# Soldann/MORB_SLAM

Hardware: AMD Instinct MI355X
Metric: stereo frames/sec ORB extract+match (752x480, 1200 feat = BASELINE configs[1]) (higher is better)
Workload: dtype u8; 1 GPU; BASELINE configs[1]: EuRoC-shaped stereo 752x480, 1200 feat: ORBextractor x2 + ComputeStereoMatches + ComputeBoW (synthetic k=10 L=6 vocabulary) + SearchByBoW vs previous frame; steps_in_flight=2, extract_streams=1, parallelism=frames dealt round-robin over 1 GPU(s)

## Files before the change

### morb_slam_amd/csrc/matcher.hip

```cpp
#include <hip/hip_runtime.h>

#include <algorithm>
#include <cstdlib>
#include <cstring>
#include <memory>
#include <vector>

#include "common.h"
#include "internal_abi.h"
#include "wave.h"
#include "extractor_internal.h"

using namespace morb;

namespace {

constexpr int TH_HIGH = 100, TH_LOW = 50, HISTO_LENGTH = 30;
constexpr int EDGE_ = 19;

struct Desc { uint32_t w[8]; };

__device__ __forceinline__ Desc load_desc(const uint8_t* p) {
  Desc d;
  const uint4* q = reinterpret_cast<const uint4*>(p);
// ... 325 lines not shown
      const int r = t / 3, c4 = (t - r * 3) * 4;
      pRow[j] = r - 5; pCol[j] = c4 - 5; pLds[j] = r * 12 + c4;
    } else {
      const int t2 = min(t, 98) - 33, r = t2 / 6, c4 = (t2 - r * 6) * 4;
      pRow[j] = r - 5; pCol[j] = c4 - 10; pLds[j] = 11 * 12 + r * 24 + c4;
    }
  }
  const uint64_t doMask = __ballot(cDo);
  const uint32_t cOffLlo = (uint32_t)cOffL, cOffLhi = (uint32_t)(cOffL >> 32), cOffRlo = (uint32_t)cOffR, cOffRhi = (uint32_t)(cOffR >> 32);
  uint8_t* patch = reinterpret_cast<uint8_t*>(pairs);
  int rS = -1, rInc = 0;
  float rD1 = 0.f, rD3 = 0.f;
  const int dy = min(lane & 15, 10);
  for (int q0 = 0; q0 < KQ; q0 += 4) {
    if (((doMask >> q0) & 15ull) == 0) continue;
    uint32_t pv[4][2];
#pragma unroll
    for (int k = 0; k < 4; ++k) {
      const int q = q0 + k;
      pv[k][0] = pv[k][1] = 0;
      if ((doMask >> q) & 1ull) {
        const unsigned long long oL = ((unsigned long long)(uint32_t)__builtin_amdgcn_readlane((int)cOffLhi, q) << 32) | (uint32_t)__builtin_amdgcn_readlane((int)cOffLlo, q);
        const unsigned long long oR = ((unsigned long long)(uint32_t)__builtin_amdgcn_readlane((int)cOffRhi, q) << 32) | (uint32_t)__builtin_amdgcn_readlane((int)cOffRlo, q);
        const int ps = __builtin_amdgcn_readlane(cPs, q);
#pragma unroll
        for (int j = 0; j < 2; ++j)
          if (pAct[j]) pv[k][j] = load_u32_unaligned(pyr + (pLeft[j] ? oL : oR) + (ptrdiff_t)pRow[j] * ps + pCol[j]);
      }
    }
    WAVE_SYNC();
#pragma unroll
    for (int k = 0; k < 4; ++k) {
      if (!((doMask >> (q0 + k)) & 1ull)) continue;
#pragma unroll
      for (int j = 0; j < 2; ++j)
        if (pAct[j]) *reinterpret_cast<uint32_t*>(patch + k * SM_PATCH + pLds[j]) = pv[k][j];
    }
    WAVE_SYNC();
#pragma unroll
    for (int k = 0; k < 4; ++k) {
      const int q = q0 + k;
      if (!((doMask >> q) & 1ull)) continue;
      const uint8_t* Lp = patch + k * SM_PATCH;
      const uint8_t* Rp = Lp + 11 * 12;
      const uint32_t l0 = *reinterpret_cast<const uint32_t*>(Lp + dy * 12), l1 = *reinterpret_cast<const uint32_t*>(Lp + dy * 12 + 4),
                     l2 = *reinterpret_cast<const uint32_t*>(Lp + dy * 12 + 8) & 0x00FFFFFFu;
      uint32_t bestKey = 0xFFFFFFFFu;
      int sums[12];
#pragma unroll
      for (int r = 0; r < 3; ++r) {
        const int sh = min(r * 4 + (lane >> 4), 10);
        const uint8_t* rp = Rp + dy * 24 + (sh & ~3);
        const uint32_t w0 = *reinterpret_cast<const uint32_t*>(rp), w1 = *reinterpret_cast<const uint32_t*>(rp + 4),
                       w2 = *reinterpret_cast<const uint32_t*>(rp + 8), w3 = *reinterpret_cast<const uint32_t*>(rp + 12);
        const uint32_t bsh = (uint32_t)(sh & 3);
        const uint32_t r0 = __builtin_amdgcn_alignbyte(w1, w0, bsh), r1 = __builtin_amdgcn_alignbyte(w2, w1, bsh),
                       r2 = __builtin_amdgcn_alignbyte(w3, w2, bsh) & 0x00FFFFFFu;
        int sv = (int)__builtin_amdgcn_sad_u8(l2, r2, __builtin_amdgcn_sad_u8(l1, r1, __builtin_amdgcn_sad_u8(l0, r0, 0u)));
        if ((lane & 15) > 10) sv = 0;
        sv += __builtin_amdgcn_update_dpp(0, sv, 0x111, 0xf, 0xf, true);
        sv += __builtin_amdgcn_update_dpp(0, sv, 0x112, 0xf, 0xf, true);
        sv += __builtin_amdgcn_update_dpp(0, sv, 0x114, 0xf, 0xf, true);
        sv += __builtin_amdgcn_update_dpp(0, sv, 0x118, 0xf, 0xf, true);
#pragma unroll
        for (int j = 0; j < 4; ++j) {
          sums[r * 4 + j] = __builtin_amdgcn_readlane(sv, 16 * j + 15);
          if (r * 4 + j < 11) {
            const uint32_t key = ((uint32_t)sums[r * 4 + j] << 4) | (uint32_t)(r * 4 + j);
            bestKey = key < bestKey ? key : bestKey;
          }
        }
      }
      const int bestS = (int)(bestKey >> 4), bi = (int)(bestKey & 15u);
      int s1 = 0, s3 = 0;
#pragma unroll
      for (int i = 0; i < 11; ++i) { s1 = (i == bi - 1) ? sums[i] : s1; s3 = (i == bi + 1) ? sums[i] : s3; }
      if (lane == q) { rS = bestS; rInc = bi - 5; rD1 = (float)s1; rD3 = (float)s3; }
    }
  }
  if (lane < KQ) {
    const int iL = iL0 + lane * 4 + wv;
    if (iL < cap) {
      float outU = -1.0f, outD = -1.0f;
      int outS = -1;
      if (cDo) {
        const int bestinc = rInc, bestS = rS;
        if (!(bestinc == -5 || bestinc == 5)) {
          const float dist1 = rD1, dist2 = (float)bestS, dist3 = rD3;
          const float deltaR = (dist1 - dist3) / (2.0f * (dist1 + dist3 - 2.0f * dist2));
          if (!(deltaR < -1 || deltaR > 1)) {
            float bestuR = sg.scale[cLvl & 15] * ((float)cUR0 + (float)bestinc + deltaR);
            float disparity = cUL - bestuR;
            if (disparity >= 0.f && disparity < maxD) {
              if (disparity <= 0) {
                disparity = 0.01f;
                bestuR = (float)((double)cUL - 0.01);
              }
              outD = mbf / disparity;
              outU = bestuR;
              outS = bestS;
            }
          }
        }
      }
      const size_t o = (size_t)f * cap + iL;
      uRight[o] = outU; depth[o] = outD; sadDist[o] = outS;
    }
  }
}

constexpr int SMED_V = 8;
template <int SMED_WAVES>
__global__ __launch_bounds__(64 * SMED_WAVES) void k_stereo_median(const int* __restrict__ count, int cap, float* __restrict__ uRight,
                                                       float* __restrict__ depth, const int* __restrict__ sadDist) {
  constexpr int NT = 64 * SMED_WAVES;
  const int f = blockIdx.x, tid = threadIdx.x;
  const int NL = count[2 * f];
  const size_t o = (size_t)f * cap;
  const bool inRegs = NL <= NT * SMED_V;
  int dv[SMED_V];
#pragma unroll
  for (int j = 0; j < SMED_V; ++j) { const int i = tid + j * NT; dv[j] = (inRegs && i < NL) ? sadDist[o + i] : -1; }
  int n = 0;
  if (inRegs) {
#pragma unroll
    for (int j = 0; j < SMED_V; ++j) n += dv[j] >= 0 ? 1 : 0;
  } else {
    for (int i = tid; i < NL; i += NT) n += sadDist[o + i] >= 0 ? 1 : 0;
  }
  __shared__ int red[2][SMED_WAVES];
  int phase = 0;
  auto blockSum = [&](int v) -> int {
    v = wave_sum(v);
    if ((tid & 63) == 0) red[phase][tid >> 6] = v;
    __syncthreads();
    int t = 0;
#pragma unroll
    for (int q = 0; q < SMED_WAVES; ++q) t += red[phase][q];
    phase ^= 1;
    return t;
  };
  const int total = blockSum(n);
  if (total == 0) return;
  const int k = total / 2;
  int lo = 0, hi = 121 * 255;
  while (lo < hi) {
    const int mid = (lo + hi) >> 1;
    int c = 0;
    if (inRegs) {
#pragma unroll
      for (int j = 0; j < SMED_V; ++j) c += (dv[j] >= 0 && dv[j] <= mid) ? 1 : 0;
    } else {
      for (int i = tid; i < NL; i += NT) { const int d = sadDist[o + i]; c += (d >= 0 && d <= mid) ? 1 : 0; }
    }
    c = blockSum(c);
    if (c > k) hi = mid; else lo = mid + 1;
  }
  const float median = (float)lo;
  const float thDist = 1.5f * 1.4f * median;
  if (inRegs) {
#pragma unroll
    for (int j = 0; j < SMED_V; ++j) {
      const int i = tid + j * NT;
      if (dv[j] >= 0 && !((float)dv[j] < thDist)) { uRight[o + i] = -1; depth[o + i] = -1; }
    }
  } else {
    for (int i = tid; i < NL; i += NT) {
      const int d = sadDist[o + i];
      if (d >= 0 && !((float)d < thDist)) { uRight[o + i] = -1; depth[o + i] = -1; }
    }
  }
}

__device__ __forceinline__ int quad_sum(int v) {
  v += __builtin_amdgcn_update_dpp(0, v, 0xB1, 0xF, 0xF, false);
  v += __builtin_amdgcn_update_dpp(0, v, 0x4E, 0xF, 0xF, false);
  return v;
}
__global__ __launch_bounds__(256) void k_bow_transform(const uint8_t* __restrict__ feat, const int* __restrict__ count,
                                                       int cap, const uint8_t* __restrict__ nodeDesc,
                                                       const int* __restrict__ firstChild, int k, int L, int levelsup,
                                                       int* __restrict__ wordId, int* __restrict__ nodeId,
                                                       const int* __restrict__ childCount) {
  const int img = blockIdx.y, t = blockIdx.x * 256 + threadIdx.x, i = t >> 2, sub = t & 3;
  if (i >= cap) return;
  const size_t o = (size_t)img * cap + i;
  if (i >= count[img]) { if (sub == 0) { wordId[o] = -1; nodeId[o] = -1; } return; }
  const uint2 d = *reinterpret_cast<const uint2*>(feat + o * 32 + sub * 8);
  const uint8_t* nd = nodeDesc + sub * 8;
  const int nid_level = L - levelsup;
  int final_id = 0, level = 0, nid = 0;
  do {
    ++level;
    const int c0 = firstChild[final_id];
    const int nc = childCount ? childCount[final_id] : k;
    int best = c0, bestd = 0x7fffffff;
    constexpr int CH = 5;
    for (int cb = c0; cb < c0 + nc; cb += CH) {
      uint2 tc[CH];
#pragma unroll
      for (int j = 0; j < CH; ++j) tc[j] = *reinterpret_cast<const uint2*>(nd + (size_t)min(cb + j, c0 + nc - 1) * 32);
#pragma unroll
      for (int j = 0; j < CH; ++j) {
        const int dd = quad_sum(__popc(d.x ^ tc[j].x) + __popc(d.y ^ tc[j].y));
        if (dd < bestd) { bestd = dd; best = min(cb + j, c0 + nc - 1); }
      }
    }
    final_id = best;
    if (level == nid_level) nid = final_id;
  } while (firstChild[final_id] >= 0);
  if (sub == 0) { wordId[o] = final_id; nodeId[o] = nid; }
}

constexpr int BT_K = 10, BT_N1 = BT_K, BT_N2 = BT_K * BT_K, BT_N3 = BT_K * BT_K * BT_K, BT_SLOTS = BT_N1 + BT_N2 + BT_N3;
template <int NLV> struct BtLds {
  static constexpr int SLOTS = NLV == 3 ? BT_SLOTS : BT_N1 + BT_N2;
  uint2 desc[SLOTS][4];
  int id[SLOTS];
  int fc[SLOTS];
  uint16_t nc[SLOTS];
};
template <int NLV>
__global__ __launch_bounds__(256) void k_bow_transform_lds(const uint8_t* __restrict__ feat, const int* __restrict__ count, int cap, int nimg,
                                                           const uint8_t* __restrict__ nodeDesc, const int* __restrict__ firstChild, int k,
                                                           int L, int levelsup, int* __restrict__ wordId, int* __restrict__ nodeId,
                                                           const int* __restrict__ childCount) {
  extern __shared__ __align__(16) uint8_t btRaw[];
  BtLds<NLV>& S = *reinterpret_cast<BtLds<NLV>*>(btRaw);
  const int tid = threadIdx.x;
  const int fc0 = firstChild[0], nc0 = childCount ? childCount[0] : k;
  auto stage = [&](int slot, int parentFc, int parentNc, int j) {
    int id = -1, fc = -1, nc = 0;
    if (parentFc >= 0 && j < parentNc) {
      id = parentFc + j;
      fc = firstChild[id];
      nc = fc >= 0 ? (childCount ? childCount[id] : k) : 0;
      const uint4* src = reinterpret_cast<const uint4*>(nodeDesc + (size_t)id * 32);
      const uint4 a = src[0], b = src[1];
      S.desc[slot][0] = make_uint2(a.x, a.y); S.desc[slot][1] = make_uint2(a.z, a.w);
      S.desc[slot][2] = make_uint2(b.x, b.y); S.desc[slot][3] = make_uint2(b.z, b.w);
    }
    S.id[slot] = id; S.fc[slot] = fc; S.nc[slot] = (uint16_t)min(nc, 0xFFFF);
  };
  if (tid < BT_N1) stage(tid, nc0 <= BT_K ? fc0 : -1, nc0, tid);
  __syncthreads();
  if (tid < BT_N2) { const int a = tid / BT_K; stage(BT_N1 + tid, S.nc[a] <= BT_K ? S.fc[a] : -1, S.nc[a], tid % BT_K); }
  __syncthreads();
  if (NLV == 3) for (int t = tid; t < BT_N3; t += 256) { const int ab = t / BT_K; stage(BT_N1 + BT_N2 + t, S.nc[BT_N1 + ab] <= BT_K ? S.fc[BT_N1 + ab] : -1, S.nc[BT_N1 + ab], t % BT_K); }
  __syncthreads();
  const int sub = tid & 3, nid_level = L - levelsup;
  const int chunksPerImg = (cap + 63) / 64, nChunks = chunksPerImg * nimg;
  const uint8_t* nd = nodeDesc + sub * 8;
  for (int ch = blockIdx.x; ch < nChunks; ch += gridDim.x) {
    const int img = ch / chunksPerImg, i = (ch - img * chunksPerImg) * 64 + (tid >> 2);
    if (i >= cap) continue;
    const size_t o = (size_t)img * cap + i;
    if (i >= count[img]) { if (sub == 0) { wordId[o] = -1; nodeId[o] = -1; } continue; }
    const uint2 d = *reinterpret_cast<const uint2*>(feat + o * 32 + sub * 8);
    int final_id = 0, level = 0, nid = 0;
    int slotBase = 0, nc = nc0, path = 0;
    bool leaf = fc0 < 0;
#pragma unroll
    for (int lv = 0; lv < NLV; ++lv) {
      if (leaf || nc > BT_K) break;
      ++level;
      int best = 0, bestd = 0x7fffffff;
      for (int j = 0; j < nc; ++j) {
        const uint2 tc = S.desc[slotBase + j][sub];
        const int dd = quad_sum(__popc(d.x ^ tc.x) + __popc(d.y ^ tc.y));
        if (dd < bestd) { bestd = dd; best = j; }
      }
      const int slot = slotBase + best;
      final_id = S.id[slot];
      if (level == nid_level) nid = final_id;
      leaf = S.fc[slot] < 0;
      nc = S.nc[slot];
      path = path * BT_K + best;
      slotBase = (lv == 0 ? BT_N1 : BT_N1 + BT_N2) + path * BT_K;
    }
    while (!leaf) {
      ++level;
      const int c0 = firstChild[final_id];
      const int ncg = childCount ? childCount[final_id] : k;
      int best = c0, bestd = 0x7fffffff;
      constexpr int CH = 5;
      for (int cb = c0; cb < c0 + ncg; cb += CH) {
        uint2 tc[CH];
#pragma unroll
        for (int j = 0; j < CH; ++j) tc[j] = *reinterpret_cast<const uint2*>(nd + (size_t)min(cb + j, c0 + ncg - 1) * 32);
#pragma unroll
        for (int j = 0; j < CH; ++j) {
          const int dd = quad_sum(__popc(d.x ^ tc[j].x) + __popc(d.y ^ tc[j].y));
          if (dd < bestd) { bestd = dd; best = min(cb + j, c0 + ncg - 1); }
        }
      }
      final_id = best;
      if (level == nid_level) nid = final_id;
      leaf = firstChild[final_id] < 0;
    }
    if (sub == 0) { wordId[o] = final_id; nodeId[o] = nid; }
  }
}

__global__ __launch_bounds__(1024) void k_bow_sort(const int* __restrict__ node, const int* __restrict__ count, int cap,
                                                   int P, unsigned long long* __restrict__ sorted) {
  extern __shared__ unsigned long long skeys[];
  const int img = blockIdx.x, tid = threadIdx.x, NT = blockDim.x;
  const int n = count[img];
  if (n == 0) {
    for (int i = tid; i < cap; i += NT) sorted[(size_t)img * cap + i] = ~0ull;
    return;
  }
  for (int i = tid; i < P; i += NT) {
    unsigned long long k = ~0ull;
    if (i < n) {
      const int nd = node[(size_t)img * cap + i];
      if (nd >= 0) k = ((unsigned long long)(unsigned)nd << 32) | (unsigned)i;
    }
    skeys[i] = k;
  }
  __syncthreads();
  const bool onePass = P / 2 <= NT;
  for (int k = 2; k <= P; k <<= 1)
    for (int j = k >> 1; j > 0; j >>= 1) {
      for (int l = tid; l < P / 2; l += NT) {
        const int i = ((l & ~(j - 1)) << 1) | (l & (j - 1)), ixj = i | j;
        const unsigned long long a = skeys[i], b = skeys[ixj];
        const bool up = (i & k) == 0;
        if ((a > b) == up) { skeys[i] = b; skeys[ixj] = a; }
      }
      const int jn = j > 1 ? j >> 1 : k;
      if (onePass && jn < 64 && j < 64) { __builtin_amdgcn_fence(__ATOMIC_SEQ_CST, "wavefront"); __builtin_amdgcn_wave_barrier(); }
      else __syncthreads();
    }
  for (int i = tid; i < cap; i += NT) sorted[(size_t)img * cap + i] = i < P ? skeys[i] : ~0ull;
}

#ifdef MORB_FAST_TIMING
__device__ unsigned long long g_bowTrace[16384 * 4];
#define BOW_MARK(k) do { if (lane == 0 && bw_ < 16384) g_bowTrace[bw_ * 4 + (k)] = wall_clock64(); } while (0)
#else
#define BOW_MARK(k)
#endif
constexpr int BM_NB = 25;
constexpr int BM_FJ = 4;
__device__ __forceinline__ unsigned wave_min_u32(unsigned v) { return morbwave::min_u32(v); }
__global__ __launch_bounds__(256) void k_bow_match(const unsigned long long* __restrict__ sortedKF,
                                                   const unsigned long long* __restrict__ sortedF,
                                                   const int* __restrict__ nKFv, const int* __restrict__ nFv, int cap,
                                                   const uint8_t* __restrict__ descKF, const uint8_t* __restrict__ hasMP,
                                                   const morb_keypoint* __restrict__ kpsKF,
                                                   const uint8_t* __restrict__ descF, const morb_keypoint* __restrict__ kpsF,
                                                   const int* __restrict__ kfImg, const int* __restrict__ fImg,
                                                   float nnratio, int* __restrict__ matchF, int* __restrict__ binF,
                                                   const int* __restrict__ nLeftv,
                                                   const uint8_t* __restrict__ hasMP2, const int* __restrict__ nValidv,
                                                   int* __restrict__ matched2) {
  extern __shared__ __align__(16) unsigned long long bowLds[];
#ifdef MORB_FAST_TIMING
  const int bw_ = (blockIdx.y * gridDim.x + blockIdx.x) * 4 + (threadIdx.x >> 6);
  if ((threadIdx.x & 63) == 0 && bw_ < 16384) g_bowTrace[bw_ * 4] = wall_clock64();
#endif
  unsigned long long* sk = bowLds;
  unsigned long long* sf = bowLds + cap;
  const int pair = blockIdx.y, tid = threadIdx.x, lane = tid & 63, wv = tid >> 6;
  const int ik = kfImg[pair], jf = fImg[pair];
  const int nKF = nKFv[ik], nF = nFv[jf];
  const bool fish = nLeftv != nullptr && nLeftv[pair] >= 0;
  const int nLeft = fish ? nLeftv[pair] : 0x7fffffff;
  const bool kfkf = hasMP2 != nullptr;
  const int nValid1 = (kfkf && nValidv) ? nValidv[ik] : 0x7fffffff, nValid2 = (kfkf && nValidv) ? nValidv[jf] : 0x7fffffff;
  const int thLow = kfkf ? TH_LOW - 1 : TH_LOW;
  {
    const unsigned long long* gk = sortedKF + (size_t)ik * cap;
    const unsigned long long* gf = sortedF + (size_t)jf * cap;
    for (int i0 = 0; i0 < cap; i0 += 256 * 4) {
      unsigned long long a[4], b[4];
#pragma unroll
      for (int k = 0; k < 4; ++k) {
        const int i = i0 + k * 256 + tid;
        a[k] = i < nKF ? gk[i] : ~0ull;
        b[k] = i < nF ? gf[i] : ~0ull;
      }
#pragma unroll
      for (int k = 0; k < 4; ++k) {
        const int i = i0 + k * 256 + tid;
        if (i < nKF) sk[i] = a[k];
        if (i < nF) sf[i] = b[k];
      }
    }
  }
  __syncthreads();
  BOW_MARK(1);
  uint16_t* starts = reinterpret_cast<uint16_t*>(sf + cap);
  __shared__ int wcnt[4];
  const uint64_t ltm = lane == 0 ? 0ull : (~0ull >> (64 - lane));
  int nStarts = 0;
  for (int i0 = 0; i0 < nKF; i0 += 256) {
    const int i = i0 + tid;
    bool st = false;
    if (i < nKF) {
      const unsigned long long k = sk[i];
      st = k != ~0ull && (i == 0 || (unsigned)(sk[i - 1] >> 32) != (unsigned)(k >> 32));
    }
    const uint64_t m = __ballot(st);
    if (lane == 0) wcnt[wv] = __popcll(m);
    __syncthreads();
    int off = nStarts;
    for (int w = 0; w < wv; ++w) off += wcnt[w];
    if (st) starts[off + __popcll(m & ltm)] = (uint16_t)i;
    nStarts += wcnt[0] + wcnt[1] + wcnt[2] + wcnt[3];
    __syncthreads();
  }
  const int G = gridDim.x * 4, g = blockIdx.x * 4 + wv;
  BOW_MARK(2);
  int* mF = matchF + (size_t)pair * cap;
  int* bF = binF + (size_t)pair * cap;
  const float factor = 1.0f / HISTO_LENGTH;
  for (int o = g; o < nStarts; o += G) {
    const int p = starts[o];
    const unsigned node = (unsigned)(sk[p] >> 32);
    int lo = 0, hi = nF;
    const unsigned long long target = (unsigned long long)node << 32;
    while (lo < hi) {
      const int mid = (lo + hi) >> 1;
      if (sf[mid] < target) lo = mid + 1; else hi = mid;
    }
    const int fBeg = lo;
    int nFs = 0;
    bool more = false;
#pragma unroll
    for (int j = 0; j < BM_FJ; ++j) {
      const int s = fBeg + j * 64 + lane;
      const uint64_t mm = __ballot(s < nF && (unsigned)(sf[s] >> 32) == node);
      nFs += __popcll(mm);
      more = mm == ~0ull;
      if (mm != ~0ull) break;
    }
    if (nFs == 0) continue;
    if (!more) {
      const int nJ = (nFs + 63) >> 6;
      int idxF[BM_FJ], myMatch[BM_FJ], myBin[BM_FJ];
      Desc dF[BM_FJ];
      float angF[BM_FJ];
#pragma unroll
      for (int j = 0; j < BM_FJ; ++j) {
        idxF[j] = 0; myMatch[j] = -1; myBin[j] = 0; angF[j] = 0.f; dF[j] = Desc{};
        if (j < nJ && j * 64 + lane < nFs) {
          idxF[j] = (int)(sf[fBeg + j * 64 + lane] & 0xFFFFFFFFu);
          dF[j] = load_desc(descF + ((size_t)jf * cap + idxF[j]) * 32);
          angF[j] = kpsF[(size_t)jf * cap + idxF[j]].angle;
          if (kfkf && (!hasMP2[(size_t)jf * cap + idxF[j]] || idxF[j] >= nValid2)) myMatch[j] = -2;
        }
      }
      for (int q0 = p; q0 < nKF; q0 += 64) {
        const uint64_t mK = __ballot(q0 + lane < nKF && (unsigned)(sk[q0 + lane] >> 32) == node);
        const int nKs = mK == ~0ull ? 64 : (int)__builtin_ctzll(~mK);
        if (nKs == 0) break;
        int idxK = 0, has = 0;
        Desc dK = {};
        float angK = 0.f;
        if (lane < nKs) {
          idxK = (int)(sk[q0 + lane] & 0xFFFFFFFFu);
          has = hasMP[(size_t)ik * cap + idxK] && idxK < nValid1;
          dK = load_desc(descKF + ((size_t)ik * cap + idxK) * 32);
          angK = kpsKF[(size_t)ik * cap + idxK].angle;
        }
        for (int q = 0; q < nKs; ++q) {
          if (!__builtin_amdgcn_readlane(has, q)) continue;
          Desc dk;
#pragma unroll
          for (int w = 0; w < 8; ++w) dk.w[w] = (uint32_t)__builtin_amdgcn_readlane((int)dK.w[w], q);
          unsigned a1 = ~0u, a2 = ~0u;
          unsigned b1 = ~0u;
#pragma unroll
          for (int j = 0; j < BM_FJ; ++j)
            if (j < nJ && j * 64 + lane < nFs && myMatch[j] == -1) {
              const unsigned key = ((unsigned)hamming(dk, dF[j]) << 16) | (unsigned)idxF[j];
              if (idxF[j] < nLeft) { if (key < a1) { a2 = a1; a1 = key; } else if (key < a2) a2 = key; }
              else if (key < b1) b1 = key;
            }
          const unsigned k1 = wave_min_u32(a1);
          const unsigned k2 = wave_min_u32(a1 == k1 ? a2 : a1);
          const unsigned r1 = fish ? wave_min_u32(b1) : ~0u;
          const int bestDist1 = k1 == ~0u ? 256 : (int)(k1 >> 16);
          const int bestDist2 = k2 == ~0u ? 256 : (int)(k2 >> 16);
          const int bestDist1R = r1 == ~0u ? 256 : (int)(r1 >> 16);
          if (bestDist1 <= thLow) {
            const int realIdxKF = __builtin_amdgcn_readlane(idxK, q);
            const float aK = __int_as_float(__builtin_amdgcn_readlane(__float_as_int(angK), q));
            const bool takeL = (float)bestDist1 < nnratio * (float)bestDist2;
            const bool takeR = bestDist1R <= TH_LOW;
            const int wantIdx = (takeL && a1 == k1) ? (int)(k1 & 0xFFFFu) : -1;
            const int wantIdxR = (takeR && b1 == r1 && r1 != ~0u) ? (int)(r1 & 0xFFFFu) : -1;
#pragma unroll
            for (int j = 0; j < BM_FJ; ++j)
              if (j < nJ && j * 64 + lane < nFs && myMatch[j] == -1 && (idxF[j] == wantIdx || idxF[j] == wantIdxR)) {
                float rot = aK - angF[j];
                if (rot < 0.0f) rot += 360.0f;
                int bin = (int)roundf(rot * factor);
                if (bin == HISTO_LENGTH) bin = 0;
                myMatch[j] = realIdxKF; myBin[j] = bin;
              }
          }
        }
        if (nKs < 64) break;
      }
#pragma unroll
      for (int j = 0; j < BM_FJ; ++j)
        if (j < nJ && j * 64 + lane < nFs && myMatch[j] >= 0) {
          if (kfkf) { mF[myMatch[j]] = idxF[j]; bF[myMatch[j]] = myBin[j]; }
          else { mF[idxF[j]] = myMatch[j]; bF[idxF[j]] = myBin[j]; }
        }
      continue;
    }
    int fEnd = fBeg;
    while (fEnd < nF && (unsigned)(sf[fEnd] >> 32) == node) ++fEnd;
    for (int q = p; q < nKF; ++q) {
      const unsigned long long kq = sk[q];
      if (kq == ~0ull || (unsigned)(kq >> 32) != node) break;
      const int realIdxKF = (int)(kq & 0xFFFFFFFFu);
      if (!hasMP[(size_t)ik * cap + realIdxKF] || realIdxKF >= nValid1) continue;
      const Desc dKF = load_desc(descKF + ((size_t)ik * cap + realIdxKF) * 32);
      unsigned long long k1 = ~0ull, k2 = ~0ull, r1 = ~0ull, r2 = ~0ull;
      for (int s0 = fBeg; s0 < fEnd; s0 += 64) {
        const int s = s0 + lane;
        if (s < fEnd) {
          const int realIdxF = (int)(sf[s] & 0xFFFFFFFFu);
          const bool cand = kfkf ? (hasMP2[(size_t)jf * cap + realIdxF] && realIdxF < nValid2 && !matched2[(size_t)pair * cap + realIdxF])
                                 : (mF[realIdxF] < 0);
          if (cand) {
            const int d = hamming(dKF, load_desc(descF + ((size_t)jf * cap + realIdxF) * 32));
            const unsigned long long key = ((unsigned long long)d << 32) | (unsigned)realIdxF;
            const bool left = realIdxF < nLeft;
            unsigned long long t1 = left ? k1 : r1, t2 = left ? k2 : r2;
            top2_insert(t1, t2, key);
            k1 = left ? t1 : k1; k2 = left ? t2 : k2; r1 = left ? r1 : t1; r2 = left ? r2 : t2;
          }
        }
      }
      wave_top2(k1, k2);
      if (fish) wave_top2(r1, r2);
      const int bestDist1 = k1 == ~0ull ? 256 : (int)(k1 >> 32);
      const int bestDist2 = k2 == ~0ull ? 256 : (int)(k2 >> 32);
      const int bestDist1R = r1 == ~0ull ? 256 : (int)(r1 >> 32);
      if (bestDist1 <= thLow) {
        const float aK = kpsKF[(size_t)ik * cap + realIdxKF].angle;
        const bool takeL = (float)bestDist1 < nnratio * (float)bestDist2, takeR = bestDist1R <= TH_LOW;
        if (lane == 0) {
          if (takeL) {
            const int bestIdxF = (int)(k1 & 0xFFFFFFFFu);
            float rot = aK - kpsF[(size_t)jf * cap + bestIdxF].angle;
            if (rot < 0.0f) rot += 360.0f;
            int bin = (int)roundf(rot * factor);
            if (bin == HISTO_LENGTH) bin = 0;
            if (kfkf) { mF[realIdxKF] = bestIdxF; bF[realIdxKF] = bin; matched2[(size_t)pair * cap + bestIdxF] = 1; }
            else { mF[bestIdxF] = realIdxKF; bF[bestIdxF] = bin; }
          }
          if (takeR) {
            const int bestIdxFR = (int)(r1 & 0xFFFFFFFFu);
            float rot = aK - kpsF[(size_t)jf * cap + bestIdxFR].angle;
            if (rot < 0.0f) rot += 360.0f;
            int bin = (int)roundf(rot * factor);
            if (bin == HISTO_LENGTH) bin = 0;
            mF[bestIdxFR] = realIdxKF; bF[bestIdxFR] = bin;
          }
        }
        __builtin_amdgcn_fence(__ATOMIC_SEQ_CST, "workgroup");
        __builtin_amdgcn_wave_barrier();
      }
    }
  }
#ifdef MORB_FAST_TIMING
  BOW_MARK(3);
#endif
}

__global__ __launch_bounds__(64) void k_distinctive(const int* __restrict__ start, const uint8_t* __restrict__ desc,
                                                    int* __restrict__ bestIdx) {
  const int mp = blockIdx.x, lane = threadIdx.x;
  const int s0 = start[mp], N = start[mp + 1] - s0;
  if (N <= 0) { if (lane == 0) bestIdx[mp] = -1; return; }
  const uint8_t* D = desc + (size_t)s0 * 32;
  const int k = (N - 1) >> 1;
  unsigned best = ~0u;
  for (int i0 = 0; i0 < N; i0 += 64) {
    const int i = i0 + lane;
    unsigned key = ~0u;
    if (i < N) {
      const Desc di = load_desc(D + (size_t)i * 32);
      int lo = 0, hi = 256;
      while (lo < hi) {
        const int mid = (lo + hi) >> 1;
        int c = 0;
        for (int j = 0; j < N; ++j) c += hamming(di, load_desc(D + (size_t)j * 32)) <= mid ? 1 : 0;
        if (c > k) hi = mid; else lo = mid + 1;
      }
      key = ((unsigned)lo << 16) | (unsigned)i;
    }
    best = key < best ? key : best;
  }
  best = wave_min_u32(best);
  if (lane == 0) bestIdx[mp] = (int)(best & 0xFFFFu);
}

__device__ void three_maxima(const int* cnt, int L, int& ind1, int& ind2, int& ind3) {
  int max1 = 0, max2 = 0, max3 = 0;
  ind1 = ind2 = ind3 = -1;
  for (int i = 0; i < L; i++) {
    const int s = cnt[i];
    if (s > max1) { max3 = max2; max2 = max1; max1 = s; ind3 = ind2; ind2 = ind1; ind1 = i; }
    else if (s > max2) { max3 = max2; max2 = s; ind3 = ind2; ind2 = i; }
    else if (s > max3) { max3 = s; ind3 = i; }
  }
  if (max2 < 0.1f * (float)max1) { ind2 = -1; ind3 = -1; }
  else if (max3 < 0.1f * (float)max1) { ind3 = -1; }
}

__global__ __launch_bounds__(256) void k_rot_filter(const int* __restrict__ nFv, const int* __restrict__ fImg, int cap,
                                                    int checkOri, int* __restrict__ matchF, const int* __restrict__ binF,
                                                    int* __restrict__ nmatches) {
  __shared__ int hist[HISTO_LENGTH];
  __shared__ int keep[3];
  __shared__ int total;
  const int pair = blockIdx.x, tid = threadIdx.x;
  const int nF = nFv[fImg[pair]];
  int* mF = matchF + (size_t)pair * cap;
  const int* bF = binF + (size_t)pair * cap;
  if (tid < HISTO_LENGTH) hist[tid] = 0;
  if (tid == 0) total = 0;
  __syncthreads();
  for (int i = tid; i < nF; i += 256)
    if (mF[i] >= 0) { atomicAdd(&total, 1); if (checkOri) atomicAdd(&hist[bF[i]], 1); }
  __syncthreads();
  if (checkOri) {
    if (tid == 0) three_maxima(hist, HISTO_LENGTH, keep[0], keep[1], keep[2]);
    __syncthreads();
    for (int i = tid; i < nF; i += 256)
// ... 64 lines not shown
}

void morb_matcher_destroy(morb_matcher* m) {
  if (!m) return;
  (void)hipSetDevice(m->device);
  (void)hipStreamSynchronize(m->stream);
  delete m;
}

int morb_matcher_device(const morb_matcher* m) { return m->device; }
void* morb_matcher_stream(const morb_matcher* m) { return (void*)m->stream; }
int morb_matcher_workspace(morb_matcher* m, int which, size_t bytes, void** out) {
  MORB_REQUIRE(m && out && which >= 0 && which < 8, MORB_ERR_INVALID, "bad workspace request");
  return m->ws[which].ensure(bytes, out);
}
int morb_matcher_const(morb_matcher* m, int slot, const void* host, size_t bytes, void** d_out, void* stream) {
  MORB_REQUIRE(m && host && d_out && slot >= 0 && slot < 4 && bytes > 0, MORB_ERR_INVALID, "bad constant-table request");
  morb_matcher::ConstSlot& c = m->consts[slot];
  int victim = 0;
  for (int w = 0; w < 4; ++w) {
    morb_matcher::ConstCopy& k = c.way[w];
    if (k.d && k.host.size() == bytes && memcmp(k.host.data(), host, bytes) == 0) { k.used = ++c.clock; *d_out = k.d; return MORB_OK; }
    if (c.way[w].used < c.way[victim].used) victim = w;
  }
  morb_matcher::ConstCopy& k = c.way[victim];
  morb::DeviceArray<> fresh;
  MORB_HIP_CHECK(fresh.alloc(bytes));
  if (k.d) m->retired.push_back(std::move(k.d));
  k.d = std::move(fresh);
  k.host.assign((const uint8_t*)host, (const uint8_t*)host + bytes);
  k.used = ++c.clock;
  hipStream_t st = stream ? (hipStream_t)stream : m->stream;
  MORB_HIP_CHECK(hipMemcpyAsync(k.d, k.host.data(), bytes, hipMemcpyHostToDevice, st));
  MORB_HIP_CHECK(hipStreamSynchronize(st));
  *d_out = k.d;
  return MORB_OK;
}
int morb_bow_sort_images(morb_matcher* m, int nimg, const int* d_node, const int* d_count, int cap, unsigned long long** d_sorted,
                         void* stream) {
  int P = 1;
  while (P < cap) P <<= 1;
  MORB_REQUIRE((size_t)P * 8 <= 160 * 1024, MORB_ERR_UNSUPPORTED, "too many features per frame for the LDS sort");
  hipStream_t st = stream ? (hipStream_t)stream : m->stream;
  unsigned long long* sortA = nullptr;
  int rc = grow(m->sortA, (size_t)nimg * cap, &sortA);
  if (rc != MORB_OK) return rc;
  MORB_HIP_CHECK(hipFuncSetAttribute(reinterpret_cast<const void*>(k_bow_sort), hipFuncAttributeMaxDynamicSharedMemorySize, P * 8));
  hipLaunchKernelGGL(k_bow_sort, dim3(nimg), dim3(P / 2 < 64 ? 64 : P / 2 > 1024 ? 1024 : P / 2), (size_t)P * 8, st, d_node, d_count, cap, P, sortA);
  *d_sorted = sortA;
  return MORB_OK;
}

size_t morb_feature_slab_bytes(int S, int cap) {
  if (S <= 0 || cap <= 0) return 0;
  return (size_t)S * cap * (sizeof(morb_keypoint) + 32 + sizeof(int)) + (size_t)S * sizeof(int);
}
namespace {
__global__ __launch_bounds__(256) void k_slab_copy(int S, int cap, const int* __restrict__ rowIdx, uint32_t* kps, uint32_t* desc, uint32_t* node, int* count,
                                                   uint32_t* slab, int dir) {
  const int f = blockIdx.x, which = blockIdx.y;
  const int row = rowIdx ? rowIdx[f] : f;
  const size_t wK = (size_t)cap * 7, wD = (size_t)cap * 8, wN = (size_t)cap;
  uint32_t* sK = slab; uint32_t* sD = sK + (size_t)S * wK; uint32_t* sN = sD + (size_t)S * wD; uint32_t* sC = sN + (size_t)S * wN;
  uint32_t *a, *b; size_t n;
  if (which == 0) { a = kps + (size_t)row * wK; b = sK + (size_t)f * wK; n = wK; }
  else if (which == 1) { a = desc + (size_t)row * wD; b = sD + (size_t)f * wD; n = wD; }
  else { a = node ? node + (size_t)row * wN : nullptr; b = sN + (size_t)f * wN; n = wN; }
  if (which == 2 && threadIdx.x == 0) { if (dir == 0) sC[f] = (uint32_t)min(max(count[row], 0), cap); else count[row] = (int)min(sC[f], (uint32_t)cap); }
  if (!a) { if (dir == 0) for (size_t i = threadIdx.x; i < n; i += 256) b[i] = 0xFFFFFFFFu; return; }
  if (dir == 0) for (size_t i = threadIdx.x; i < n; i += 256) b[i] = a[i];
  else for (size_t i = threadIdx.x; i < n; i += 256) a[i] = b[i];
}
}
int morb_feature_slab_pack(morb_matcher* m, int S, int cap, const int* d_rows, const morb_keypoint* d_kps, const uint8_t* d_desc, const int* d_node,
                           const int* d_count, void* d_slab, void* stream) {
  MORB_REQUIRE(m && S > 0 && cap > 0 && d_kps && d_desc && d_count && d_slab, MORB_ERR_INVALID, "bad argument");
  MORB_HIP_CHECK(hipSetDevice(m->device));
  hipStream_t st = stream ? (hipStream_t)stream : m->stream;
  hipLaunchKernelGGL(k_slab_copy, dim3(S, 3), dim3(256), 0, st, S, cap, d_rows, (uint32_t*)d_kps, (uint32_t*)d_desc, (uint32_t*)d_node, (int*)d_count,
                     (uint32_t*)d_slab, 0);
  MORB_HIP_CHECK(hipGetLastError());
  return MORB_OK;
}
int morb_feature_slab_unpack(morb_matcher* m, int S, int cap, const void* d_slab, const int* d_rows, morb_keypoint* d_kps, uint8_t* d_desc, int* d_node,
                             int* d_count, void* stream) {
  MORB_REQUIRE(m && S > 0 && cap > 0 && d_kps && d_desc && d_count && d_slab, MORB_ERR_INVALID, "bad argument");
  MORB_HIP_CHECK(hipSetDevice(m->device));
  hipStream_t st = stream ? (hipStream_t)stream : m->stream;
  hipLaunchKernelGGL(k_slab_copy, dim3(S, 3), dim3(256), 0, st, S, cap, d_rows, (uint32_t*)d_kps, (uint32_t*)d_desc, (uint32_t*)d_node, d_count,
                     (uint32_t*)const_cast<void*>(d_slab), 1);
  MORB_HIP_CHECK(hipGetLastError());
  return MORB_OK;
}

int morb_hamming_pairs(morb_matcher* m, const uint8_t* d_a, const uint8_t* d_b, int n, int* d_out, void* stream) {
  MORB_REQUIRE(m && d_a && d_b && d_out && n >= 0, MORB_ERR_INVALID, "bad argument");
  MORB_HIP_CHECK(hipSetDevice(m->device));
  hipStream_t st = stream ? (hipStream_t)stream : m->stream;
  if (n) hipLaunchKernelGGL(k_hamming_pairs, dim3(div_up(n, 256)), dim3(256), 0, st, d_a, d_b, n, d_out);
  MORB_HIP_CHECK(hipGetLastError());
  return MORB_OK;
}

int morb_hamming_knn2_batch(morb_matcher* m, int nprob, const uint8_t* d_query, const int* d_nq, int qPitch,
                            const int* d_qOff, const uint8_t* d_train, const int* d_nt, int tPitch, const int* d_tOff,
                            int* d_idx, int* d_dist, void* stream) {
  MORB_REQUIRE(m && d_query && d_train && d_nq && d_nt && d_idx && d_dist, MORB_ERR_INVALID, "NULL argument");
  MORB_REQUIRE(nprob > 0 && qPitch > 0 && tPitch > 0, MORB_ERR_INVALID, "bad sizes");
  MORB_HIP_CHECK(hipSetDevice(m->device));
  hipStream_t st = stream ? (hipStream_t)stream : m->stream;
  hipLaunchKernelGGL(k_knn2, dim3(div_up(qPitch, 256), nprob), dim3(256), 0, st, d_query, d_nq, qPitch, d_train, d_nt,
                     tPitch, d_qOff, d_tOff, d_idx, d_dist);
  MORB_HIP_CHECK(hipGetLastError());
  return MORB_OK;
}

int morb_stereo_match_batch(morb_matcher* m, const morb_extractor* e, int nframes, const morb_keypoint* d_kps,
                            const uint8_t* d_desc, const int* d_count, int cap, float mbf, float mb, float* d_uRight,
                            float* d_depth, void* stream) {
  MORB_REQUIRE(m && e && d_kps && d_desc && d_count && d_uRight && d_depth, MORB_ERR_INVALID, "NULL argument");
  MORB_REQUIRE(nframes > 0 && cap > 0 && mb > 0.f, MORB_ERR_INVALID, "bad sizes");
  MORB_REQUIRE(e->W > 0 && e->nimgLast >= 2 * nframes, MORB_ERR_INVALID,
               "the extractor must have processed the 2*nframes images (left = 2f, right = 2f+1) of this batch");
  MORB_REQUIRE(e->device == m->device, MORB_ERR_INVALID, "extractor and matcher live on different devices");
  MORB_HIP_CHECK(hipSetDevice(m->device));
  hipStream_t st = stream ? (hipStream_t)stream : m->stream;
  int* sad = nullptr;
  uint8_t* stereoRec = nullptr;
  int rc = grow(m->sad, (size_t)nframes * cap, &sad);
  if (rc != MORB_OK) return rc;
  StereoGeom sg = {};
  for (int l = 0; l < 16; ++l) {
    const LevelGeom& g = e->geom[l < e->nlevels ? l : e->nlevels - 1];
    sg.pyrOff[l] = g.pyrOff; sg.pyrImg[l] = g.pyrImg; sg.pstride[l] = g.pstride; sg.w[l] = g.w;
    sg.scale[l] = e->scale[l < e->nlevels ? l : e->nlevels - 1]; sg.invScale[l] = e->invScale[l < e->nlevels ? l : e->nlevels - 1];
  }
  sg.nRows = e->geom[0].h;
  const StereoRec ro = stereo_rec(cap);
  rc = grow(m->stereoRec, (size_t)nframes * ro.bytes, &stereoRec);
  if (rc != MORB_OK) return rc;
  const size_t prepSmem = (size_t)ro.bytes + SM_MAXB * sizeof(int);
  const size_t stereoSmem = (size_t)ro.bytes + 4 * SM_KQ * (32 + 8) + 4 * SM_PCAP * sizeof(uint32_t);
  MORB_REQUIRE(prepSmem <= 160 * 1024 && stereoSmem <= 160 * 1024 && cap < 65536 && e->nlevels <= 16, MORB_ERR_UNSUPPORTED, "too many keypoints per image for the LDS-resident right-keypoint table");
  MORB_HIP_CHECK(hipFuncSetAttribute(reinterpret_cast<const void*>(k_stereo_prep), hipFuncAttributeMaxDynamicSharedMemorySize, (int)prepSmem));
  MORB_HIP_CHECK(hipFuncSetAttribute(reinterpret_cast<const void*>(k_stereo_match), hipFuncAttributeMaxDynamicSharedMemorySize, (int)stereoSmem));
  const int lk = sm_lk_for(nframes);
  hipLaunchKernelGGL(k_stereo_prep, dim3(nframes), dim3(nframes <= 16 ? 1024 : 256), prepSmem, st, sg, d_kps, d_count, cap, stereoRec);
  hipLaunchKernelGGL(k_stereo_match, dim3(div_up(cap, lk), nframes), dim3(256), stereoSmem, st, sg, e->d_pyr, d_kps, d_desc,
                     d_count, cap, mbf, mb, d_uRight, d_depth, sad, lk, stereoRec);
  if (nframes <= 16) hipLaunchKernelGGL(k_stereo_median<16>, dim3(nframes), dim3(64 * 16), 0, st, d_count, cap, d_uRight, d_depth, sad);
  else hipLaunchKernelGGL(k_stereo_median<4>, dim3(nframes), dim3(64 * 4), 0, st, d_count, cap, d_uRight, d_depth, sad);
  MORB_HIP_CHECK(hipGetLastError());
  return MORB_OK;
}

namespace {
int launch_bow_transform(hipStream_t st, int nimg, const uint8_t* d_desc, const int* d_count, int cap, const uint8_t* d_nodeDesc,
                         const int* d_firstChild, int k, int kmax, int L, int levelsup, int* d_wordId, int* d_nodeId, const int* d_childCount) {
  const int nChunks = div_up(cap, 64) * nimg;
  const char* sv = getenv("MORB_BOW_STAGE");
  if (sv && kmax <= BT_K && nChunks >= 64) {
    const int nlv = atoi(sv);
    const char* gv = getenv("MORB_BOW_GRID");
    const int grid = std::min(nChunks, gv ? atoi(gv) : 1024);
    if (nlv == 3) {
      MORB_HIP_CHECK(hipFuncSetAttribute(reinterpret_cast<const void*>(k_bow_transform_lds<3>), hipFuncAttributeMaxDynamicSharedMemorySize, (int)sizeof(BtLds<3>)));
      hipLaunchKernelGGL(k_bow_transform_lds<3>, dim3(grid), dim3(256), sizeof(BtLds<3>), st, d_desc, d_count, cap, nimg, d_nodeDesc, d_firstChild, k, L,
                         levelsup, d_wordId, d_nodeId, d_childCount);
    } else {
      hipLaunchKernelGGL(k_bow_transform_lds<2>, dim3(grid), dim3(256), sizeof(BtLds<2>), st, d_desc, d_count, cap, nimg, d_nodeDesc, d_firstChild, k, L,
                         levelsup, d_wordId, d_nodeId, d_childCount);
    }
  } else {
    hipLaunchKernelGGL(k_bow_transform, dim3(div_up(4 * cap, 256), nimg), dim3(256), 0, st, d_desc, d_count, cap, d_nodeDesc, d_firstChild, k, L,
                       levelsup, d_wordId, d_nodeId, d_childCount);
  }
  MORB_HIP_CHECK(hipGetLastError());
  return MORB_OK;
}
}

int morb_bow_transform_batch(morb_matcher* m, int nimg, const uint8_t* d_desc, const int* d_count, int cap,
                             const uint8_t* d_nodeDesc, const int* d_firstChild, int k, int L, int levelsup,
                             int* d_wordId, int* d_nodeId, void* stream) {
  MORB_REQUIRE(m && d_desc && d_count && d_nodeDesc && d_firstChild && d_wordId && d_nodeId, MORB_ERR_INVALID, "NULL argument");
  MORB_REQUIRE(nimg > 0 && cap > 0 && k > 0 && L > 0, MORB_ERR_INVALID, "bad sizes");
  MORB_HIP_CHECK(hipSetDevice(m->device));
  hipStream_t st = stream ? (hipStream_t)stream : m->stream;
  return launch_bow_transform(st, nimg, d_desc, d_count, cap, d_nodeDesc, d_firstChild, k, k, L, levelsup, d_wordId, d_nodeId, nullptr);
}

int morb_bow_transform_tree_batch(morb_matcher* m, int nimg, const uint8_t* d_desc, const int* d_count, int cap,
                                  const uint8_t* d_nodeDesc, const int* d_firstChild, const int* d_childCount, int L, int levelsup,
                                  int* d_wordId, int* d_nodeId, void* stream) {
  MORB_REQUIRE(m && d_desc && d_count && d_nodeDesc && d_firstChild && d_childCount && d_wordId && d_nodeId, MORB_ERR_INVALID,
               "NULL argument");
  MORB_REQUIRE(nimg > 0 && cap > 0 && L > 0, MORB_ERR_INVALID, "bad sizes");
  MORB_HIP_CHECK(hipSetDevice(m->device));
  hipStream_t st = stream ? (hipStream_t)stream : m->stream;
  return launch_bow_transform(st, nimg, d_desc, d_count, cap, d_nodeDesc, d_firstChild, 0, BT_K, L, levelsup, d_wordId, d_nodeId, d_childCount);
}

struct morb_vocabulary {
  int k = 0, L = 0, scoring = 0, weighting = 0;
  std::vector<uint8_t> desc;
  std::vector<int> firstChild;
  std::vector<int> childCount;
  std::vector<int> parent;
  std::vector<int> wordId;
  std::vector<double> weight;
};

int morb_vocabulary_load_text(const char* path, morb_vocabulary** out) {
  MORB_REQUIRE(path && out, MORB_ERR_INVALID, "NULL argument");
  *out = nullptr;
  FILE* f = fopen(path, "r");
  MORB_REQUIRE(f, MORB_ERR_INVALID, "cannot open the vocabulary file");
  std::unique_ptr<morb_vocabulary> v(new morb_vocabulary());
  int n1 = 0, n2 = 0;
  if (fscanf(f, "%d %d %d %d", &v->k, &v->L, &n1, &n2) != 4 || v->k < 0 || v->k > 20 || v->L < 1 || v->L > 10 || n1 < 0 || n1 > 5 ||
      n2 < 0 || n2 > 3) {
    fclose(f);
    set_error("Vocabulary loading failure: This is not a correct text file!");
    return MORB_ERR_INVALID;
  }
  v->scoring = n1; v->weighting = n2;
  v->desc.assign(32, 0); v->firstChild.assign(1, -1); v->childCount.assign(1, 0); v->parent.assign(1, -1); v->wordId.assign(1, -1);
  v->weight.assign(1, 0.0);
  int nWords = 0;
  for (;;) {
    int pid = 0, isLeaf = 0;
    if (fscanf(f, "%d %d", &pid, &isLeaf) != 2) break;
    const int nid = (int)v->parent.size();
    int d[32];
    bool ok = pid >= 0 && pid < nid;
    for (int i = 0; i < 32 && ok; ++i) ok = fscanf(f, "%d", &d[i]) == 1;
    double w = 0;
    if (ok) ok = fscanf(f, "%lf", &w) == 1;
    if (!ok) { fclose(f); set_error("malformed vocabulary node %d", nid); return MORB_ERR_INVALID; }
    v->parent.push_back(pid);
    for (int i = 0; i < 32; ++i) v->desc.push_back((uint8_t)d[i]);
    v->weight.push_back((double)w);
    v->firstChild.push_back(-1); v->childCount.push_back(0);
    v->wordId.push_back(isLeaf > 0 ? nWords++ : -1);
    if (v->childCount[pid] == 0) v->firstChild[pid] = nid;
    else if (v->firstChild[pid] + v->childCount[pid] != nid) {
      fclose(f);
      set_error("children of vocabulary node %d are not contiguous", pid);
      return MORB_ERR_UNSUPPORTED;
    }
    v->childCount[pid]++;
  }
  fclose(f);
  *out = v.release();
  return MORB_OK;
}
void morb_vocabulary_destroy(morb_vocabulary* v) { delete v; }
int morb_vocabulary_info(const morb_vocabulary* v, int* k, int* L, int* nNodes, int* nWords) {
  MORB_REQUIRE(v, MORB_ERR_INVALID, "NULL vocabulary");
  if (k) *k = v->k;
  if (L) *L = v->L;
  if (nNodes) *nNodes = (int)v->parent.size();
  if (nWords) { int n = 0; for (int w : v->wordId) n += w >= 0; *nWords = n; }
  return MORB_OK;
}
int morb_vocabulary_arrays(const morb_vocabulary* v, uint8_t* nodeDesc, int* firstChild, int* childCount, int* wordId, float* weight) {
  MORB_REQUIRE(v, MORB_ERR_INVALID, "NULL vocabulary");
  const size_t n = v->parent.size();
  if (nodeDesc) memcpy(nodeDesc, v->desc.data(), n * 32);
  if (firstChild) memcpy(firstChild, v->firstChild.data(), n * sizeof(int));
  if (childCount) memcpy(childCount, v->childCount.data(), n * sizeof(int));
  if (wordId) memcpy(wordId, v->wordId.data(), n * sizeof(int));
  if (weight) for (size_t i = 0; i < n; ++i) weight[i] = (float)v->weight[i];
  return MORB_OK;
}

int morb_vocabulary_weights(const morb_vocabulary* v, double* weight, int* scoring, int* weighting) {
  MORB_REQUIRE(v, MORB_ERR_INVALID, "NULL vocabulary");
  if (weight) memcpy(weight, v->weight.data(), v->weight.size() * sizeof(double));
  if (scoring) *scoring = v->scoring;
  if (weighting) *weighting = v->weighting;
  return MORB_OK;
}

static int search_by_bow_impl(morb_matcher* m, int npairs, const int* d_kfImg, const int* d_fImg, int nimg,
                              const morb_keypoint* d_kps, const uint8_t* d_desc, const int* d_node, const int* d_count,
                              const uint8_t* d_hasMP, int cap, float nnratio, int checkOri, int* d_matchF,
                              int* d_nmatches, const int* d_nLeft, void* stream, const uint8_t* d_hasMP2 = nullptr,
                              const int* d_nValid = nullptr) {
  MORB_REQUIRE(m && d_kfImg && d_fImg && d_kps && d_desc && d_node && d_count && d_hasMP && d_matchF && d_nmatches,
               MORB_ERR_INVALID, "NULL argument");
  MORB_REQUIRE(npairs > 0 && nimg > 0 && cap > 0, MORB_ERR_INVALID, "bad sizes");
  int P = 1;
  while (P < cap) P <<= 1;
  MORB_REQUIRE((size_t)P * 8 <= 160 * 1024, MORB_ERR_UNSUPPORTED, "too many features per frame for the LDS sort");
  MORB_HIP_CHECK(hipSetDevice(m->device));
  hipStream_t st = stream ? (hipStream_t)stream : m->stream;
  unsigned long long* sortA = nullptr;
  int* bin = nullptr;
  int rc = grow(m->sortA, (size_t)nimg * cap, &sortA);
  if (rc != MORB_OK) return rc;
  rc = grow(m->bin, (size_t)npairs * cap, &bin);
  if (rc != MORB_OK) return rc;
  MORB_HIP_CHECK(hipFuncSetAttribute(reinterpret_cast<const void*>(k_bow_sort), hipFuncAttributeMaxDynamicSharedMemorySize, P * 8));
  hipLaunchKernelGGL(k_bow_sort, dim3(nimg), dim3(P / 2 < 64 ? 64 : P / 2 > 1024 ? 1024 : P / 2), (size_t)P * 8, st, d_node, d_count, cap, P, sortA);
  const size_t nm = (size_t)npairs * cap;
  hipLaunchKernelGGL(k_fill_i32, dim3((unsigned)((nm + 255) / 256)), dim3(256), 0, st, d_matchF, nm, -1);
  int* matched2 = nullptr;
  if (d_hasMP2) {
    void* w = nullptr;
    rc = morb_matcher_workspace(m, 7, sizeof(int) * nm, &w);
    if (rc != MORB_OK) return rc;
    matched2 = (int*)w;
    hipLaunchKernelGGL(k_fill_i32, dim3((unsigned)((nm + 255) / 256)), dim3(256), 0, st, matched2, nm, 0);
  }
  MORB_REQUIRE(cap < 65536 && (size_t)cap * 18 <= 160 * 1024, MORB_ERR_UNSUPPORTED, "too many features per frame for the LDS-resident node tables");
  MORB_HIP_CHECK(hipFuncSetAttribute(reinterpret_cast<const void*>(k_bow_match), hipFuncAttributeMaxDynamicSharedMemorySize, (int)((size_t)cap * 18)));
  hipLaunchKernelGGL(k_bow_match, dim3(BM_NB, npairs), dim3(256), (size_t)cap * 18, st, sortA, sortA, d_count, d_count,
                     cap, d_desc, d_hasMP, d_kps, d_desc, d_kps, d_kfImg, d_fImg, nnratio, d_matchF, bin, d_nLeft, d_hasMP2,
                     d_nValid, matched2);
  hipLaunchKernelGGL(k_rot_filter, dim3(npairs), dim3(256), 0, st, d_count, d_hasMP2 ? d_kfImg : d_fImg, cap, checkOri, d_matchF,
                     bin, d_nmatches);
  MORB_HIP_CHECK(hipGetLastError());
  return MORB_OK;
}

int morb_search_by_bow_batch(morb_matcher* m, int npairs, const int* d_kfImg, const int* d_fImg, int nimg,
                             const morb_keypoint* d_kps, const uint8_t* d_desc, const int* d_node, const int* d_count,
                             const uint8_t* d_hasMP, int cap, float nnratio, int checkOri, int* d_matchF,
                             int* d_nmatches, void* stream) {
  return search_by_bow_impl(m, npairs, d_kfImg, d_fImg, nimg, d_kps, d_desc, d_node, d_count, d_hasMP, cap, nnratio, checkOri,
                            d_matchF, d_nmatches, nullptr, stream);
}

int morb_distinctive_descriptors_batch(morb_matcher* m, int nMP, const int* d_start, const uint8_t* d_desc, int* d_bestIdx,
                                       void* stream) {
  MORB_REQUIRE(m && d_start && d_desc && d_bestIdx && nMP >= 0, MORB_ERR_INVALID, "bad argument");
  MORB_HIP_CHECK(hipSetDevice(m->device));
  hipStream_t st = stream ? (hipStream_t)stream : m->stream;
  if (nMP) hipLaunchKernelGGL(k_distinctive, dim3(nMP), dim3(64), 0, st, d_start, d_desc, d_bestIdx);
  MORB_HIP_CHECK(hipGetLastError());
  return MORB_OK;
}

int morb_search_by_bow_kfkf_batch(morb_matcher* m, int npairs, const int* d_kf1Img, const int* d_kf2Img, const int* d_nValid, int nimg,
                                  const morb_keypoint* d_kps, const uint8_t* d_desc, const int* d_node, const int* d_count,
                                  const uint8_t* d_hasMP, int cap, float nnratio, int checkOri, int* d_match12, int* d_nmatches,
                                  void* stream) {
  return search_by_bow_impl(m, npairs, d_kf1Img, d_kf2Img, nimg, d_kps, d_desc, d_node, d_count, d_hasMP, cap, nnratio, checkOri,
                            d_match12, d_nmatches, nullptr, stream, d_hasMP, d_nValid);
}

int morb_search_by_bow_fisheye_batch(morb_matcher* m, int npairs, const int* d_kfImg, const int* d_fImg, const int* d_nLeft,
                                     int nimg, const morb_keypoint* d_kps, const uint8_t* d_desc, const int* d_node,
                                     const int* d_count, const uint8_t* d_hasMP, int cap, float nnratio, int checkOri,
                                     int* d_matchF, int* d_nmatches, void* stream) {
  MORB_REQUIRE(d_nLeft, MORB_ERR_INVALID, "NULL argument");
  return search_by_bow_impl(m, npairs, d_kfImg, d_fImg, nimg, d_kps, d_desc, d_node, d_count, d_hasMP, cap, nnratio, checkOri,
                            d_matchF, d_nmatches, d_nLeft, stream);
}

#ifdef MORB_FAST_TIMING
int morb_bow_timing(unsigned long long* out, int reset) {
  (void)reset;
  MORB_HIP_CHECK(hipMemcpyFromSymbol(out, HIP_SYMBOL(g_bowTrace), sizeof(unsigned long long) * 16384 * 4));
  return 0;
}
#endif

}
```

Measured before the change: 137,100 frames/s.

## Replace bitonic BoW node sort with single-wave counting sort

```diff
diff --git a/morb_slam_amd/csrc/matcher.hip b/morb_slam_amd/csrc/matcher.hip
--- a/morb_slam_amd/csrc/matcher.hip
+++ b/morb_slam_amd/csrc/matcher.hip
@@ -651,10 +651,9 @@
   }
 }
 
-__global__ __launch_bounds__(1024) void k_bow_sort(const int* __restrict__ node, const int* __restrict__ count, int cap,
-                                                   int P, unsigned long long* __restrict__ sorted) {
-  extern __shared__ unsigned long long skeys[];
-  const int img = blockIdx.x, tid = threadIdx.x, NT = blockDim.x;
+__device__ __forceinline__ void bow_sort_image(const int* __restrict__ node, const int* __restrict__ count, int cap, int P,
+                                               unsigned long long* __restrict__ sorted, unsigned long long* skeys, int img) {
+  const int tid = threadIdx.x, NT = blockDim.x;
   const int n = count[img];
   if (n == 0) {
     for (int i = tid; i < cap; i += NT) sorted[(size_t)img * cap + i] = ~0ull;
@@ -683,6 +682,77 @@
       else __syncthreads();
     }
   for (int i = tid; i < cap; i += NT) sorted[(size_t)img * cap + i] = i < P ? skeys[i] : ~0ull;
+}
+__global__ __launch_bounds__(1024) void k_bow_sort(const int* __restrict__ node, const int* __restrict__ count, int cap,
+                                                   int P, unsigned long long* __restrict__ sorted) {
+  extern __shared__ unsigned long long skeys[];
+  bow_sort_image(node, count, cap, P, sorted, skeys, blockIdx.x);
+}
+constexpr int CS_NB = 2048;
+__global__ __launch_bounds__(64) void k_bow_csort(const int* __restrict__ node, const int* __restrict__ count, int cap, int P,
+                                                  unsigned long long* __restrict__ sorted) {
+  extern __shared__ unsigned long long csLds[];
+  int* cursor = reinterpret_cast<int*>(csLds);
+  const int img = blockIdx.x, lane = threadIdx.x;
+  const int n = min(count[img], cap);
+  if (n <= 0) return;
+  const int* nd = node + (size_t)img * cap;
+  unsigned long long* out = sorted + (size_t)img * cap;
+  unsigned mn = ~0u, mx = 0;
+  int nv = 0;
+  for (int i = lane; i < n; i += 64) {
+    const int v = nd[i];
+    if (v >= 0) { mn = min(mn, (unsigned)v); mx = max(mx, (unsigned)v); ++nv; }
+  }
+  mn = morbwave::min_u32(mn);
+  mx = ~morbwave::min_u32(~mx);
+  nv = morbwave::sum_i32(nv);
+  if (nv > 0 && mx - mn >= (unsigned)CS_NB) { bow_sort_image(node, count, cap, P, sorted, csLds, img); return; }
+  if (nv > 0) {
+    const int range = (int)(mx - mn) + 1;
+    const int nbits = 32 - __builtin_clz((unsigned)range);
+    for (int b = lane; b < range; b += 64) cursor[b] = 0;
+    __builtin_amdgcn_fence(__ATOMIC_SEQ_CST, "wavefront");
+    __builtin_amdgcn_wave_barrier();
+    for (int i = lane; i < n; i += 64) {
+      const int v = nd[i];
+      if (v >= 0) atomicAdd(&cursor[v - (int)mn], 1);
+    }
+    __builtin_amdgcn_fence(__ATOMIC_SEQ_CST, "wavefront");
+    __builtin_amdgcn_wave_barrier();
+    const int per = (range + 63) >> 6, b0 = lane * per, b1 = min(b0 + per, range);
+    int s = 0;
+    for (int b = b0; b < b1; ++b) s += cursor[b];
+    int incl = s;
+    MORB_DPP_SCAN(incl, 0, morbwave::op_add);
+    int run = incl - s;
+    for (int b = b0; b < b1; ++b) { const int c = cursor[b]; cursor[b] = run; run += c; }
+    __builtin_amdgcn_fence(__ATOMIC_SEQ_CST, "wavefront");
+    __builtin_amdgcn_wave_barrier();
+    const uint64_t ltm = lane == 0 ? 0ull : (~0ull >> (64 - lane));
+    for (int i0 = 0; i0 < n; i0 += 64) {
+      const int i = i0 + lane;
+      const int v = i < n ? nd[i] : -1;
+      const bool valid = v >= 0;
+      const unsigned key = valid ? (unsigned)v - mn : 0u;
+      uint64_t peers = __ballot(valid);
+      for (int bit = 0; bit < nbits; ++bit) {
+        const uint64_t m = __ballot((key >> bit) & 1u);
+        peers &= ((key >> bit) & 1u) ? m : ~m;
+      }
+      int base = 0;
+      if (valid) base = cursor[key];
+      __builtin_amdgcn_fence(__ATOMIC_SEQ_CST, "wavefront");
+      __builtin_amdgcn_wave_barrier();
+      if (valid) {
+        out[base + __popcll(peers & ltm)] = ((unsigned long long)(unsigned)v << 32) | (unsigned)i;
+        if ((peers & ~(ltm | (1ull << lane))) == 0) cursor[key] = base + __popcll(peers);
+      }
+      __builtin_amdgcn_fence(__ATOMIC_SEQ_CST, "wavefront");
+      __builtin_amdgcn_wave_barrier();
+    }
+  }
+  for (int i = nv + lane; i < cap; i += 64) out[i] = ~0ull;
 }
 
 #ifdef MORB_FAST_TIMING
@@ -1353,8 +1423,9 @@
   if (rc != MORB_OK) return rc;
   rc = grow(m->bin, (size_t)npairs * cap, &bin);
   if (rc != MORB_OK) return rc;
-  MORB_HIP_CHECK(hipFuncSetAttribute(reinterpret_cast<const void*>(k_bow_sort), hipFuncAttributeMaxDynamicSharedMemorySize, P * 8));
-  hipLaunchKernelGGL(k_bow_sort, dim3(nimg), dim3(P / 2 < 64 ? 64 : P / 2 > 1024 ? 1024 : P / 2), (size_t)P * 8, st, d_node, d_count, cap, P, sortA);
+  const int csLds = std::max(CS_NB * (int)sizeof(int), P * 8);
+  MORB_HIP_CHECK(hipFuncSetAttribute(reinterpret_cast<const void*>(k_bow_csort), hipFuncAttributeMaxDynamicSharedMemorySize, csLds));
+  hipLaunchKernelGGL(k_bow_csort, dim3(nimg), dim3(64), (size_t)csLds, st, d_node, d_count, cap, P, sortA);
   const size_t nm = (size_t)npairs * cap;
   hipLaunchKernelGGL(k_fill_i32, dim3((unsigned)((nm + 255) / 256)), dim3(256), 0, st, d_matchF, nm, -1);
   int* matched2 = nullptr;
```

Measured after the change: 138,400 frames/s (median of 4 runs). Within noise of the previous version (+0.9%).
